# yeeus/GCI

Hardware: AMD Instinct MI355X
Metric: aligned Gbases/s through filter+depth pipeline (CHM13, 40x HiFi) (higher is better)
Workload: dtype int32

## Files before the change

### gci_amd/build.py

```python
from __future__ import annotations

import os
import subprocess

_HERE = os.path.dirname(os.path.abspath(__file__))
CSRC = os.path.join(_HERE, "csrc")
LIB = os.path.join(CSRC, "libgci_hip.so")
SOURCES = [os.path.join(CSRC, f) for f in ("api_ctx.hip", "k_filter.hip", "k_join.hip", "k_depth.hip", "k_track.hip", "k_bedgraph.hip", "k_hist.hip", "k_depth_parse.hip", "k_sdepth.hip", "k_deflate.hip", "k_depth_gz.hip", "k_paf.hip", "k_inflate.hip", "k_inflate_wave.hip", "k_records.hip", "k_pages.hip", "k_cover.hip", "k_shard.hip", "k_hbm.hip", "host_io.cpp", "staging.cpp")]
DEPS = SOURCES + [os.path.join(CSRC, "gci_common.h"), os.path.join(CSRC, "gci_ctx.hpp"), os.path.join(CSRC, "gci_wave.hpp"),
                  os.path.join(CSRC, "gci_text_tiles.hpp"), os.path.join(CSRC, "gci_crc_gf2.hpp"), os.path.join(CSRC, "gci_deflate_codes.hpp"),
                  os.path.join(_HERE, "..", "include", "gci_hip.h")]


def hipcc() -> str:
    for c in (os.environ.get("HIPCC"), "/opt/rocm/bin/hipcc", "hipcc"):
        if c and (os.path.sep not in c or os.path.exists(c)):
            return c
    raise RuntimeError("hipcc not found")


def needs_build() -> bool:
    if not os.path.exists(LIB):
        return True
    t = os.path.getmtime(LIB)
    return any(os.path.getmtime(d) > t for d in DEPS)
# ... 32 lines not shown
```

### gci_amd/csrc/api_ctx.hip

```cpp
#include "gci_ctx.hpp"
#include <stdlib.h>
#include <vector>

int gci_fail(gci_ctx* c, hipError_t e, const char* what)
{
    if (c) c->err = std::string(what) + ": " + hipGetErrorString(e);
    return GCI_E_HIP;
}

int gci_ensure(gci_ctx* ctx, DevBuf& b, size_t bytes)
{
    if (bytes <= b.cap) return GCI_OK;
    if (b.p) { HIPCHK(hipStreamSynchronize(ctx->stream)); HIPCHK(gci_dfree(b.p)); b.p = nullptr; b.cap = 0; }
    size_t want = bytes + bytes / 4 + 256;
    HIPCHK(gci_dmalloc(ctx->device, &b.p, want));
    b.cap = want;
    return GCI_OK;
}

int gci_upload_small(gci_ctx* ctx, void* d_dst, const void* h_src, size_t bytes)
{
    HIPCHK(hipStreamSynchronize(ctx->stream));
    if (bytes > ctx->h_pinned_cap) {
        if (ctx->h_pinned) HIPCHK(hipHostFree(ctx->h_pinned));
// ... 6 lines not shown
    memcpy(ctx->h_pinned, h_src, bytes);
    HIPCHK(hipMemcpyAsync(d_dst, ctx->h_pinned, bytes, hipMemcpyHostToDevice, ctx->stream));
    return GCI_OK;
}

extern "C" int gci_abi_version(void) { return GCI_ABI_VERSION; }

extern "C" int gci_ctx_create(int device, void* stream, int own_stream, gci_ctx** out)
{
    if (!out) return GCI_E_INVALID;
    gci_ctx* ctx = new (std::nothrow) gci_ctx();
    if (!ctx) return GCI_E_NOMEM;
    ctx->device = device;
    { const char* fd = getenv("GCI_FORCE_DENSE"); if (fd && fd[0] == '1') ctx->sparse_max = -1; }
    { const char* m = getenv("GCI_JOIN"); ctx->join_mode = m && m[0] == 'c' ? 1 : m && m[0] == 'p' ? 2 : 0; }
    { const char* g = getenv("GCI_PAGES_GRID"); const long n = g ? atol(g) : 0; ctx->pg_grid_cap = n > 0 && n < (1 << 20) ? (uint32_t)n : 0u; }
    hipError_t e = hipSetDevice(device);
    if (e != hipSuccess) { delete ctx; return GCI_E_HIP; }
    if (!own_stream) { ctx->stream = (hipStream_t)stream; }
    else {
        e = hipStreamCreateWithFlags(&ctx->stream, hipStreamNonBlocking);
        if (e != hipSuccess) { delete ctx; return GCI_E_HIP; }
        ctx->own_stream = true;
    }
    {
        uint32_t lut[TEXT_LUT];
        gci_text_lut_host(lut);
        if (gci_dmalloc(device, &ctx->text_lut.p, sizeof lut) != hipSuccess ||
            hipMemcpy(ctx->text_lut.p, lut, sizeof lut, hipMemcpyHostToDevice) != hipSuccess) {
            gci_ctx_destroy(ctx);
// ... 187 lines not shown
```

### gci_amd/csrc/gci_ctx.hpp

```cpp
#pragma once
#include <hip/hip_runtime.h>
#include <stdint.h>
#include <stdlib.h>
#include <string.h>
#include <string>
#include <vector>

#include "../../include/gci_hip.h"
#include "gci_common.h"
#include "gci_wave.hpp"

#define TILE GCI_TILE
#define TEXT_LUT 1000
#define BLOCK 256
static_assert(TILE == BLOCK * 16, "a tile is 16 elements per thread");

constexpr int GCI_RUN_MAX = 64;
constexpr uint32_t GCI_RUNS_WALK = 0xFFFFFFFFu;

struct DevBuf {
    void* p = nullptr;
    size_t cap = 0;
};

// ... 4 lines not shown
    std::string err;
    int32_t n_contigs = 0;
    std::vector<int64_t> len, off;
    std::vector<int64_t> tile_first;
    int64_t total = 0, n_tiles = 0;
    DevBuf d_len, d_off, d_tile_first;
    DevBuf tile_cd;
    DevBuf tile_carry;
    DevBuf evt_off;
    DevBuf d_tile_valid;
    DevBuf dense_flag;
    DevBuf dense_list;
    int32_t sparse_max = 62;
    bool join_dirty = false;
    int join_mode = 0;
    uint32_t k1_parity = 0;
    int cd_state = 0;
    int counted_flank = 0;
    bool count_deferred = false;
    DevBuf evp_items, evp_hist, evp_blk;
    DevBuf events;
    DevBuf blk_a, blk_b;
    DevBuf tile_sum;
    DevBuf tile_u32, tile_u64, blk_u64;
    uint32_t build_max_n = 0;
    int build_flank = 0;
    bool build_pending = false, build_text = false;
    bool build_runs_wanted = false;
    DevBuf build_nruns, build_runs;
    const void* build_runs_track = nullptr;
// ... 413 lines not shown
```

### gci_amd/csrc/k_join.hip

```cpp
#include "gci_ctx.hpp"
#include <stdlib.h>

struct JoinFiles {
    gci_join_file f[GCI_MAX_JOIN_FILES];
    int n;
};

#define SLOT_EMPTY 0xFFFFFFFFFFFFFFFFull

__device__ __forceinline__ const uint8_t* name_ptr(const gci_join_file& f, uint32_t idx)
{
    return f.d_name_base + f.d_name_off[idx] + f.name_delta;
}

__device__ __forceinline__ bool same_name(const JoinFiles& F, int fa, uint32_t ia, const gci_rec& a,
                                          unsigned long long owner)
{
    const int fb = (int)(owner >> 32);
    const uint32_t ib = (uint32_t)owner;
    const gci_rec& b = F.f[fb].d_recs[ib];
    if (a.name_hash != b.name_hash || a.name_len != b.name_len) return false;
    const uint8_t* pa = name_ptr(F.f[fa], ia);
    const uint8_t* pb = name_ptr(F.f[fb], ib);
    for (uint32_t i = 0; i < a.name_len; i++) if (pa[i] != pb[i]) return false;
// ... 145 lines not shown
        }
    }
}



struct __attribute__((aligned(16))) PartEntry {
    unsigned long long key;
    uint32_t idx;
    uint32_t meta;
    int32_t start, end, qlen;
    uint32_t name_off16;
};
static_assert(sizeof(PartEntry) == 32, "partition entry is 32 bytes");
#define PART_CHUNK 8192
#define PART_CONTIG_BITS 26
#define PART_KEY_MASK 0xFFFFFFFFFFFFull
#define PART_CMP_MASK 0x0FFFFFFFFFFFFFFFull
#define PART_MAX_NAME 4095u
#define PART_WIN (1ull << 63)
#define PART_NONE 0xFFFFFFFFu
struct PartFiles { uint32_t chunk_first[GCI_MAX_JOIN_FILES + 1]; };

__device__ __forceinline__ bool part_takes(const gci_rec& r)
{
    return (r.flags & GCI_REC_PASS) && !((uint32_t)r.contig >> PART_CONTIG_BITS) && r.name_len <= PART_MAX_NAME;
}

__device__ __forceinline__ void part_refuse(unsigned long long* status)
{
// ... 30 lines not shown
    return e;
}

__global__ __launch_bounds__(BLOCK) void k_part1_hist(JoinFiles F, PartFiles P, int shift, uint32_t n_bins, uint32_t n_chunks,
                                                      uint32_t* __restrict__ hist, uint32_t* __restrict__ reset_n_out,
                                                      unsigned long long* __restrict__ status)
{
    __shared__ uint32_t h[256];
    const uint32_t t = threadIdx.x, chunk = blockIdx.x;
    if (chunk == 0 && t == 0) *reset_n_out = 0;
    h[t] = 0;
    __syncthreads();
    const int f = part_file_of(P, F.n, chunk);
    const uint32_t i0 = (chunk - P.chunk_first[f]) * PART_CHUNK, n = F.f[f].n_recs;
    const gci_rec* __restrict__ recs = F.f[f].d_recs;
#pragma unroll 4
    for (int k = 0; k < PART_CHUNK / BLOCK; k++) {
        const uint32_t i = i0 + k * BLOCK + t;
        if (i < n) {
            const gci_rec r = recs[i];
            if (part_takes(r)) atomicAdd(&h[(uint32_t)((r.name_hash & PART_KEY_MASK) >> shift) & (n_bins - 1)], 1u);
            else if (r.flags & GCI_REC_PASS) part_refuse(status);
        }
    }
    __syncthreads();
    if (t < n_bins) hist[(size_t)t * n_chunks + chunk] = h[t];
}

#define SC_TILE 1024
#define SC_PER (SC_TILE / BLOCK)
struct ScatterLds {
    int4 stage[SC_TILE * 2];
    uint32_t tcnt[256], toff[256], gofs[256], cnt[256], base[256];
    uint32_t wtot[BLOCK / 64], total;
    uint8_t sbin[SC_TILE];
// ... 42 lines not shown
__global__ __launch_bounds__(BLOCK) void k_part1_scatter(JoinFiles F, PartFiles P, int shift, uint32_t n_bins, uint32_t n_chunks,
                                                         const uint32_t* __restrict__ off, PartEntry* __restrict__ out,
                                                         unsigned long long* __restrict__ status)
{
    __shared__ ScatterLds L;
    const uint32_t t = threadIdx.x, chunk = blockIdx.x;
    L.cnt[t] = 0; L.tcnt[t] = 0;
    L.base[t] = t < n_bins ? off[(size_t)t * n_chunks + chunk] : 0u;
    __syncthreads();
    const int f = part_file_of(P, F.n, chunk);
    const uint32_t i0 = (chunk - P.chunk_first[f]) * PART_CHUNK, n = F.f[f].n_recs;
    const gci_rec* __restrict__ recs = F.f[f].d_recs;
    const uint64_t* __restrict__ noff = F.f[f].d_name_off;
    const uint64_t delta = F.f[f].name_delta;
    for (uint32_t tile = 0; tile < PART_CHUNK && i0 + tile < n; tile += SC_TILE) {
        PartEntry e[SC_PER];
        int d[SC_PER];
#pragma unroll
        for (int k = 0; k < SC_PER; k++) {
            const uint32_t i = i0 + tile + k * BLOCK + t;
            d[k] = -1;
            e[k].key = 0; e[k].idx = 0; e[k].meta = 0; e[k].start = e[k].end = e[k].qlen = 0; e[k].name_off16 = 0;
            if (i < n) {
                const gci_rec r = recs[i];
                if (part_takes(r)) {
                    const uint64_t at = noff[i] + delta;
                    if (at >> 36) part_refuse(status);
                    e[k].key = (r.name_hash & PART_KEY_MASK) | ((unsigned long long)r.name_len << 48) | ((unsigned long long)(at & 15ull) << 60);
                    e[k].idx = i;
                    e[k].meta = (uint32_t)r.contig | ((uint32_t)f << PART_CONTIG_BITS) | ((r.flags & GCI_REC_HQ) ? 1u << 30 : 0u) |
                                ((r.flags & GCI_REC_NAME16) ? 1u << 31 : 0u);
                    e[k].start = r.start; e[k].end = r.end; e[k].qlen = r.qlen;
                    e[k].name_off16 = (uint32_t)(at >> 4);
                    d[k] = (int)((uint32_t)((e[k].key & PART_KEY_MASK) >> shift) & (n_bins - 1));
                }
            }
        }
        scatter_tile(L, e, d, n_bins, out, (int)t);
    }
}

__global__ __launch_bounds__(BLOCK) void k_part_mid(const uint32_t* __restrict__ off1, uint32_t n_bins, uint32_t n_chunks,
                                                    uint32_t* __restrict__ seg)
{
    __shared__ uint32_t s[257], c[257];
    const uint32_t t = threadIdx.x;
    if (t <= n_bins) s[t] = off1[(size_t)t * n_chunks];
    if (t == 0 && n_bins == 256) s[256] = off1[(size_t)256 * n_chunks];
    __syncthreads();
    if (t == 0) {
        uint32_t acc = 0;
        for (uint32_t d = 0; d < n_bins; d++) { c[d] = acc; acc += (s[d + 1] - s[d] + PART_CHUNK - 1) / PART_CHUNK; }
        c[n_bins] = acc;
    }
    __syncthreads();
    if (t <= n_bins) { seg[t] = s[t]; seg[n_bins + 1 + t] = c[t]; }
    if (t == 0 && n_bins == 256) { seg[256] = s[256]; seg[513] = c[256]; }
}

__device__ __forceinline__ bool part2_chunk(const uint32_t* sS, const uint32_t* sC, uint32_t n_seg, uint32_t w, uint32_t& j,
                                            uint32_t& k, uint32_t& a, uint32_t& b, uint32_t& nch)
{
    if (w >= sC[n_seg]) return false;
    uint32_t lo = 0, hi = n_seg;
    while (hi - lo > 1) { const uint32_t mid = (lo + hi) >> 1; if (sC[mid] <= w) lo = mid; else hi = mid; }
    j = lo; k = w - sC[j]; nch = sC[j + 1] - sC[j];
    a = sS[j] + k * PART_CHUNK;
    b = min(sS[j + 1], a + PART_CHUNK);
    return true;
}

__global__ __launch_bounds__(BLOCK) void k_part2_hist(const PartEntry* __restrict__ in, const uint32_t* __restrict__ seg,
                                                      uint32_t n_seg, int shift, uint32_t n_bins, uint32_t* __restrict__ hist)
{
    __shared__ uint32_t sS[257], sC[257], h[256];
    const uint32_t t = threadIdx.x, w = blockIdx.x;
    for (uint32_t i = t; i <= n_seg; i += BLOCK) { sS[i] = seg[i]; sC[i] = seg[n_seg + 1 + i]; }
    h[t] = 0;
    __syncthreads();
    uint32_t j, k, a, b, nch;
    if (!part2_chunk(sS, sC, n_seg, w, j, k, a, b, nch)) {
        if (t < n_bins) hist[(size_t)w * n_bins + t] = 0;
        return;
    }
    for (uint32_t i = a + t; i < b; i += BLOCK)
        atomicAdd(&h[(uint32_t)((in[i].key & PART_KEY_MASK) >> shift) & (n_bins - 1)], 1u);
    __syncthreads();
    if (t < n_bins) hist[(size_t)sC[j] * n_bins + (size_t)t * nch + k] = h[t];
}

__global__ __launch_bounds__(BLOCK) void k_part2_scatter(const PartEntry* __restrict__ in, const uint32_t* __restrict__ seg,
                                                         uint32_t n_seg, int shift, uint32_t n_bins,
                                                         const uint32_t* __restrict__ off, PartEntry* __restrict__ out)
{
    __shared__ ScatterLds L;
    __shared__ uint32_t sS[257], sC[257];
    const uint32_t t = threadIdx.x, w = blockIdx.x;
    for (uint32_t i = t; i <= n_seg; i += BLOCK) { sS[i] = seg[i]; sC[i] = seg[n_seg + 1 + i]; }
    L.cnt[t] = 0; L.tcnt[t] = 0;
    __syncthreads();
    uint32_t j, k, a, b, nch;
    if (!part2_chunk(sS, sC, n_seg, w, j, k, a, b, nch)) return;
    L.base[t] = t < n_bins ? off[(size_t)sC[j] * n_bins + (size_t)t * nch + k] : 0u;
    __syncthreads();
    for (uint32_t tile = a; tile < b; tile += SC_TILE) {
        PartEntry e[SC_PER];
        int d[SC_PER];
#pragma unroll
        for (int q = 0; q < SC_PER; q++) {
            const uint32_t i = tile + q * BLOCK + t;
            d[q] = -1;
            e[q].key = 0; e[q].idx = 0; e[q].meta = 0; e[q].start = e[q].end = e[q].qlen = 0; e[q].name_off16 = 0;
            if (i < b) {
                e[q] = load_entry(in + i);
                d[q] = (int)((uint32_t)((e[q].key & PART_KEY_MASK) >> shift) & (n_bins - 1));
            }
        }
        scatter_tile(L, e, d, n_bins, out, (int)t);
    }
}

__device__ __forceinline__ bool names_equal(const uint8_t* __restrict__ pa, const uint8_t* __restrict__ pb, uint32_t len)
{
    const uint32_t sa = (uint32_t)((uintptr_t)pa & 3u), sb = (uint32_t)((uintptr_t)pb & 3u);
    const uint32_t* __restrict__ qa = reinterpret_cast<const uint32_t*>(pa - sa);
    const uint32_t* __restrict__ qb = reinterpret_cast<const uint32_t*>(pb - sb);
    const uint32_t na = (sa + len + 3u) >> 2, nb = (sb + len + 3u) >> 2;
    uint32_t diff = 0;
    for (uint32_t w0 = 0; 4u * w0 < len; w0 += 8) {
        uint32_t a[9], b[9];
#pragma unroll
        for (int k = 0; k < 9; k++) {
// ... 19 lines not shown
    const uint32_t s = (uint32_t)((uintptr_t)pa & 15u);
    const uint4* __restrict__ qa = reinterpret_cast<const uint4*>(pa - s);
    const uint4* __restrict__ qb = reinterpret_cast<const uint4*>(pb - s);
    const uint32_t end = s + len;
    const uint4 z = make_uint4(0, 0, 0, 0);
    const uint4 a0 = qa[0], b0 = qb[0];
    const uint4 a1 = end > 16 ? qa[1] : z, b1 = end > 16 ? qb[1] : z;
    const uint4 a2 = end > 32 ? qa[2] : z, b2 = end > 32 ? qb[2] : z;
    uint32_t d = (s ? 0u : a0.x ^ b0.x) | (a0.y ^ b0.y) | (a0.z ^ b0.z) | (a0.w ^ b0.w);
    d |= (a1.x ^ b1.x) | (a1.y ^ b1.y) | (a1.z ^ b1.z) | (a1.w ^ b1.w);
    d |= (a2.x ^ b2.x) | (a2.y ^ b2.y) | (a2.z ^ b2.z) | (a2.w ^ b2.w);
    return d == 0;
}

struct PartJoinArgs {
    const PartEntry* in; const uint32_t* seg; const uint32_t* off2;
    uint32_t n_seg, n_bins2, slots, slot_shift;
};

template <bool CLAIM>
__device__ __forceinline__ uint32_t part_probe(unsigned long long* meta, uint32_t S, uint32_t slot_shift, const PartEntry& e, uint32_t i,
                                               const PartEntry* __restrict__ in, const JoinFiles& F, bool exact, uint16_t* used,
                                               uint32_t* s_used)
{
    const unsigned long long tag = e.key & 0xFFFFFFFFFFull;
    uint32_t slot = (uint32_t)((e.key & PART_KEY_MASK) >> slot_shift) & (S - 1);
    for (uint32_t probes = 0; probes < S; probes++) {
        unsigned long long m = meta[slot];
        if (m == SLOT_EMPTY) {
            if (!CLAIM) return PART_NONE;
            m = atomicCAS(meta + slot, SLOT_EMPTY, (tag << 24) | ((unsigned long long)i << 1));
            if (m == SLOT_EMPTY) {
                used[atomicAdd(s_used, 1u)] = (uint16_t)slot;
                return slot;
            }
        }
        if ((m >> 24) == tag) {
            if (!exact) return slot;
            const uint32_t c = (uint32_t)(m >> 1) & 0x7FFFFFu;
            if (c == i) return slot;
            const PartEntry ce = load_entry(in + c);
            if (((ce.key ^ e.key) & PART_CMP_MASK) == 0 &&
                names_equal(entry_name(F, e), entry_name(F, ce), (uint32_t)(e.key >> 48) & 0xFFFu))
                return slot;
        }
        slot = (slot + 1) & (S - 1);
    }
    return PART_NONE;
}

// ... 109 lines not shown
                else { s = ms; e = me; }
            } else have = false;
        } else {
            have = true; contig = r_contig; s = r.y; e = r.z;
        }
    }
    if (!have) return false;
    if (contig_map) { contig = contig_map[contig]; if (contig < 0) return false; }
    o.contig = contig; o.start = s; o.end = e; o.pad = 0;
    return true;
}

#ifndef PART_E
#define PART_E 2
#endif
#ifndef JB
#define JB 512
#endif
template <int FN>
__global__ __launch_bounds__(JB) __attribute__((amdgpu_waves_per_eu(4, 4))) void k_join_part(JoinFiles F, PartJoinArgs A, double ovlp_percent,
                                                     const int32_t* __restrict__ contig_map, gci_ivl* __restrict__ sparse,
                                                     uint32_t* __restrict__ bucket_cnt, uint32_t* __restrict__ bucket_lo,
                                                     unsigned long long* __restrict__ status, const CountArgs cnt)
{
    extern __shared__ __attribute__((aligned(16))) unsigned long long sm[];
    __shared__ uint32_t wtot[JB / 64];
    __shared__ uint32_t s_used, s_bad;
    __shared__ int64_t s_len[COUNT_LDS], s_tf[COUNT_LDS];
    const uint32_t S = A.slots;
    const int Fn = FN ? FN : F.n;
    unsigned long long* meta = sm;
    unsigned long long* cname = sm + S;
    unsigned long long* last = sm + 2 * (size_t)S;
    int4* pay = reinterpret_cast<int4*>(sm + 2 * (size_t)S + (size_t)S * Fn);
    uint16_t* used = reinterpret_cast<uint16_t*>(sm + 2 * (size_t)S + 3 * (size_t)S * Fn);
    const int t = threadIdx.x, lane = t & 63, wave = t >> 6;
    const uint32_t j = blockIdx.x / A.n_bins2, d = blockIdx.x % A.n_bins2;
    const uint32_t cj = A.seg[A.n_seg + 1 + j], nch = A.seg[A.n_seg + 2 + j] - cj;
    if (nch == 0) { if (t == 0) bucket_cnt[blockIdx.x] = 0u; return; }
    const uint32_t lo = A.off2[(size_t)cj * A.n_bins2 + (size_t)d * nch], hi = A.off2[(size_t)cj * A.n_bins2 + (size_t)(d + 1) * nch];
    if (t == 0) { bucket_cnt[blockIdx.x] = 0u; bucket_lo[blockIdx.x] = lo; }
    if (lo == hi) return;
    const bool tables_in_lds = cnt.tile_cd && cnt.n_contigs <= COUNT_LDS;
    if (tables_in_lds) for (int c = t; c < cnt.n_contigs; c += JB) { s_len[c] = cnt.len[c]; s_tf[c] = cnt.tile_first[c]; }
    const PartEntry* __restrict__ in = A.in + lo;
    const uint32_t n = hi - lo;
    if (n >> 23) {
        if (t == 0) part_refuse(status);
        return;
    }
    const uint32_t cmask = (1u << PART_CONTIG_BITS) - 1u;
    const bool in_regs = n <= PART_E * JB;
    PartEntry ent[PART_E];
    uint32_t slot_of[PART_E];
#pragma unroll
    for (int k = 0; k < PART_E; k++) {
        slot_of[k] = PART_NONE;
        const uint32_t i = (uint32_t)t + (uint32_t)k * JB;
        if (in_regs && i < n) ent[k] = load_entry(in + i);
        else { ent[k].key = 0; ent[k].idx = 0; ent[k].meta = 0; ent[k].start = ent[k].end = ent[k].qlen = 0; ent[k].name_off16 = 0; }
    }
    auto name_word = [](const PartEntry& e) -> unsigned long long {
        return (unsigned long long)e.name_off16 | ((e.key >> 60) << 32) | (((e.key >> 48) & 0xFFFull) << 36) |
               ((unsigned long long)((e.meta >> PART_CONTIG_BITS) & 15u) << 48) | ((unsigned long long)(e.meta >> 31) << 52);
    };
    auto insert = [&](const PartEntry& e, uint32_t i, bool exact) -> uint32_t {
        const uint32_t slot = part_probe<true>(meta, S, A.slot_shift, e, i, in, F, exact, used, &s_used);
        if (slot == PART_NONE) { part_refuse(status); return slot; }
        if (((uint32_t)(meta[slot] >> 1) & 0x7FFFFFu) == i) cname[slot] = name_word(e);
        const int file = (int)((e.meta >> PART_CONTIG_BITS) & 15u);
        const unsigned long long ord = (((unsigned long long)(e.meta & cmask) << 32) | e.idx) + 1ull;
        atomicMax(last + (size_t)slot * Fn + file, ord);
        if (Fn > 1 && (e.meta >> 30 & 1u)) atomicOr(meta + slot, 1ull);
        return slot;
    };
    auto settle = [&](const PartEntry& e, uint32_t i, uint32_t slot, bool exact) {
        const int file = (int)((e.meta >> PART_CONTIG_BITS) & 15u);
        const unsigned long long ord = (((unsigned long long)(e.meta & cmask) << 32) | e.idx) + 1ull;
        if (last[(size_t)slot * Fn + file] == ord) {
            last[(size_t)slot * Fn + file] = PART_WIN | i;
            pay[(size_t)slot * Fn + file] = make_int4((int)(e.meta & cmask), e.start, e.end, e.qlen);
        }
// ... 2 lines not shown
            const uint32_t len = (uint32_t)(e.key >> 48) & 0xFFFu;
            const uint8_t* cn = F.f[(cw >> 48) & 15u].d_name_base + (((cw & 0xFFFFFFFFull) << 4) | ((cw >> 32) & 15ull));
            const uint8_t* mn = entry_name(F, e);
            bool same;
            if (((uint32_t)(cw >> 36) & 0xFFFu) != len) same = false;
            else if ((e.meta >> 31) && ((cw >> 52) & 1ull) && len <= 44u && (((uintptr_t)mn ^ (uintptr_t)cn) & 15u) == 0)
                same = names_equal16(mn, cn, len);
            else same = names_equal(mn, cn, len);
            if (!same) s_bad = 1u;
        }
    };
    bool exact = false;
    for (;;) {
        for (uint32_t s = t; s < S; s += JB) meta[s] = SLOT_EMPTY;
        for (uint32_t s = t; s < S * (uint32_t)Fn; s += JB) last[s] = 0ull;
        if (t == 0) { s_used = 0; s_bad = 0; }
        __syncthreads();
        if (in_regs) {
#pragma unroll
            for (int k = 0; k < PART_E; k++) {
                const uint32_t i = (uint32_t)t + (uint32_t)k * JB;
                if (i < n) slot_of[k] = insert(ent[k], i, exact);
            }
        } else {
            for (uint32_t i = t; i < n; i += JB) insert(load_entry(in + i), i, exact);
        }
        __syncthreads();
        if (in_regs) {
#pragma unroll
            for (int k = 0; k < PART_E; k++) {
                const uint32_t i = (uint32_t)t + (uint32_t)k * JB;
                if (i < n && slot_of[k] != PART_NONE) settle(ent[k], i, slot_of[k], exact);
            }
        } else {
            for (uint32_t i = t; i < n; i += JB) {
                const PartEntry e = load_entry(in + i);
                const uint32_t slot = part_probe<false>(meta, S, A.slot_shift, e, i, in, F, exact, used, &s_used);
                if (slot != PART_NONE) settle(e, i, slot, exact);
            }
        }
        __syncthreads();
        if (exact || !s_bad) break;
        exact = true;
        __syncthreads();
    }
    auto fold_one = [&](const PartEntry& e, uint32_t i, uint32_t slot, gci_ivl& keep) -> bool {
        const int file = (int)((e.meta >> PART_CONTIG_BITS) & 15u);
        if (last[(size_t)slot * Fn + file] != (PART_WIN | i)) return false;
        for (int f = 0; f < file; f++) if (last[(size_t)slot * Fn + f] != 0) return false;
        return fold_from_entry<FN>(F, in, e, file, slot, last, pay, (meta[slot] & 1ull) != 0, ovlp_percent, contig_map, status, keep);
    };
    auto emit = [&](const gci_ivl& keep, uint32_t w) {
// ... 20 lines not shown
        uint32_t pre = inc - mine, all = 0;
#pragma unroll
        for (int w = 0; w < JB / 64; w++) { if (w < wave) pre += wtot[w]; all += wtot[w]; }
        if (t == 0) bucket_cnt[blockIdx.x] = all;
        uint32_t w = pre;
#pragma unroll
        for (int k = 0; k < PART_E; k++) if (ok[k]) emit(keep[k], w++);
    } else {
        uint32_t run = 0;
        for (uint32_t i0 = 0; i0 < n; i0 += JB) {
            const uint32_t i = i0 + t;
            gci_ivl keep;
            bool ok = false;
            if (i < n) {
                const PartEntry e = load_entry(in + i);
                const uint32_t slot = part_probe<false>(meta, S, A.slot_shift, e, i, in, F, exact, used, &s_used);
                ok = slot != PART_NONE && fold_one(e, i, slot, keep);
            }
            const unsigned long long bal = __ballot(ok);
            if (lane == 0) wtot[wave] = (uint32_t)__builtin_popcountll(bal);
            __syncthreads();
            uint32_t pre = (uint32_t)__builtin_popcountll(bal & ((1ull << lane) - 1ull)), all = 0;
#pragma unroll
            for (int w = 0; w < JB / 64; w++) { if (w < wave) pre += wtot[w]; all += wtot[w]; }
            if (ok) emit(keep, run + pre);
            run += all;
            __syncthreads();
        }
        if (t == 0) bucket_cnt[blockIdx.x] = run;
    }
}

__global__ __launch_bounds__(BLOCK) void k_join_gather(const gci_ivl* __restrict__ sparse, const uint32_t* __restrict__ bucket_cnt,
                                                       const uint32_t* __restrict__ bucket_lo, const uint32_t* __restrict__ off,
                                                       uint32_t n_buckets, gci_ivl* __restrict__ out, uint32_t cap, uint32_t* __restrict__ n_out)
{
    const uint32_t b = blockIdx.x * (BLOCK / 64) + (threadIdx.x >> 6), lane = threadIdx.x & 63;
    if (blockIdx.x == 0 && threadIdx.x == 0) *n_out = off[n_buckets];
    if (b >= n_buckets) return;
    const uint32_t c = bucket_cnt[b];
    if (!c) return;
    const gci_ivl* __restrict__ src = sparse + bucket_lo[b];
    const uint32_t o = off[b];
    for (uint32_t r = lane; r < c; r += 64) if (o + r < cap) out[o + r] = src[r];
}

static int name_join_partitioned(gci_ctx* ctx, const JoinFiles& F, uint64_t total, double ovlp_percent,
                                 const int32_t* d_contig_map, gci_ivl* d_out, uint32_t cap, uint32_t* d_n_out,
                                 uint64_t* d_status, const CountArgs& cnt, bool* done)
{
    *done = false;
    uint32_t S = 1024;
    while (S > 128 && (size_t)S * (16 + 24 * (size_t)F.n) > 65536) S >>= 1;
    uint64_t nb = 256;
    while (nb * S * 5 < total * 8) nb <<= 1;
    if (nb > 65536) return GCI_OK;
    int bits = 0;
    while ((1ull << bits) < nb) bits++;
    const int b1 = (bits + 1) / 2, b2 = bits - b1;
    const uint32_t B1 = 1u << b1, B2 = 1u << b2;
    int s_bits = 0;
    while ((1u << s_bits) < S) s_bits++;
    const int shift1 = 48 - b1, shift2 = 48 - b1 - b2, slot_shift = shift2 - s_bits;
    PartFiles P;
    uint32_t C1 = 0;
    for (int f = 0; f < F.n; f++) { P.chunk_first[f] = C1; C1 += (F.f[f].n_recs + PART_CHUNK - 1) / PART_CHUNK; }
    for (int f = F.n; f <= GCI_MAX_JOIN_FILES; f++) P.chunk_first[f] = C1;
    const uint32_t C2 = (uint32_t)(total / PART_CHUNK) + B1 + 1;
    const size_t n1 = (size_t)B1 * C1, n2 = (size_t)C2 * B2;
    GCI_TRY(gci_ensure(ctx, ctx->part_a, total * sizeof(PartEntry) + 16));
    GCI_TRY(gci_ensure(ctx, ctx->part_b, total * sizeof(PartEntry) + 16));
    GCI_TRY(gci_ensure(ctx, ctx->part_hist, (n1 + 1 + n2 + 1 + 2 * (size_t)B1 + 2) * 4 + 64));
    GCI_TRY(gci_ensure(ctx, ctx->part_blk, ((n1 > n2 ? n1 : n2) / TILE + 2) * 4));
    uint32_t* hist1 = (uint32_t*)ctx->part_hist.p;
    uint32_t* hist2 = hist1 + n1 + 1;
    uint32_t* seg = hist2 + n2 + 1;
    PartEntry* pa = (PartEntry*)ctx->part_a.p;
    PartEntry* pb = (PartEntry*)ctx->part_b.p;
    HIPCHK(hipMemsetAsync(d_status, 0xFF, 8, ctx->stream));
    {
        ProfScope _ps(ctx, GCI_PROF_PARTITION);
        hipLaunchKernelGGL(k_part1_hist, dim3(C1), dim3(BLOCK), 0, ctx->stream, F, P, shift1, B1, C1, hist1, d_n_out,
                           (unsigned long long*)d_status);
        LAUNCHCHK("k_part1_hist");
        int r = device_exclusive_scan<uint32_t, uint32_t>(ctx, hist1, hist1, (uint32_t*)ctx->part_blk.p, (int64_t)n1, true);
        if (r) return r;
        hipLaunchKernelGGL(k_part1_scatter, dim3(C1), dim3(BLOCK), 0, ctx->stream, F, P, shift1, B1, C1, (const uint32_t*)hist1, pa,
                           (unsigned long long*)d_status);
        LAUNCHCHK("k_part1_scatter");
        hipLaunchKernelGGL(k_part_mid, dim3(1), dim3(BLOCK), 0, ctx->stream, (const uint32_t*)hist1, B1, C1, seg);
        LAUNCHCHK("k_part_mid");
        hipLaunchKernelGGL(k_part2_hist, dim3(C2), dim3(BLOCK), 0, ctx->stream, (const PartEntry*)pa, (const uint32_t*)seg, B1,
                           shift2, B2, hist2);
        LAUNCHCHK("k_part2_hist");
        r = device_exclusive_scan<uint32_t, uint32_t>(ctx, hist2, hist2, (uint32_t*)ctx->part_blk.p, (int64_t)n2, true);
        if (r) return r;
        hipLaunchKernelGGL(k_part2_scatter, dim3(C2), dim3(BLOCK), 0, ctx->stream, (const PartEntry*)pa, (const uint32_t*)seg, B1,
                           shift2, B2, (const uint32_t*)hist2, pb);
        LAUNCHCHK("k_part2_scatter");
    }
    {
        ProfScope _ps(ctx, GCI_PROF_JOIN_PART);
        PartJoinArgs A;
        A.in = pb; A.seg = seg; A.off2 = hist2; A.n_seg = B1; A.n_bins2 = B2; A.slots = S; A.slot_shift = (uint32_t)slot_shift;
        const size_t lds = (size_t)S * (16 + 24 * (size_t)F.n) + (size_t)S * 2;
        const dim3 grid(B1 * B2), block(JB);
        const uint32_t NB = B1 * B2;
        GCI_TRY(gci_ensure(ctx, ctx->join_bucket, ((size_t)3 * NB + 2) * 4 + 64));
        uint32_t* bcnt = (uint32_t*)ctx->join_bucket.p;
        uint32_t* blo = bcnt + NB;
        uint32_t* boff = blo + NB;
        gci_ivl* sparse = (gci_ivl*)pa;
        static_assert(sizeof(gci_ivl) <= sizeof(PartEntry), "the sparse intervals fit the partition buffer");
        const void* kfn = F.n == 1 ? (const void*)k_join_part<1> : F.n == 2 ? (const void*)k_join_part<2> : F.n == 3 ? (const void*)k_join_part<3>
                        : F.n == 4 ? (const void*)k_join_part<4> : (const void*)k_join_part<0>;
        HIPCHK(hipFuncSetAttribute(kfn, hipFuncAttributeMaxDynamicSharedMemorySize, (int)lds));
        switch (F.n) {
        case 1: hipLaunchKernelGGL((k_join_part<1>), grid, block, lds, ctx->stream, F, A, ovlp_percent, d_contig_map, sparse, bcnt, blo, (unsigned long long*)d_status, cnt); break;
        case 2: hipLaunchKernelGGL((k_join_part<2>), grid, block, lds, ctx->stream, F, A, ovlp_percent, d_contig_map, sparse, bcnt, blo, (unsigned long long*)d_status, cnt); break;
        case 3: hipLaunchKernelGGL((k_join_part<3>), grid, block, lds, ctx->stream, F, A, ovlp_percent, d_contig_map, sparse, bcnt, blo, (unsigned long long*)d_status, cnt); break;
        case 4: hipLaunchKernelGGL((k_join_part<4>), grid, block, lds, ctx->stream, F, A, ovlp_percent, d_contig_map, sparse, bcnt, blo, (unsigned long long*)d_status, cnt); break;
        default: hipLaunchKernelGGL((k_join_part<0>), grid, block, lds, ctx->stream, F, A, ovlp_percent, d_contig_map, sparse, bcnt, blo, (unsigned long long*)d_status, cnt); break;
        }
        LAUNCHCHK("k_join_part");
        int r2 = device_exclusive_scan<uint32_t, uint32_t>(ctx, bcnt, boff, (uint32_t*)ctx->part_blk.p, (int64_t)NB, true);
        if (r2) return r2;
        hipLaunchKernelGGL(k_join_gather, dim3((NB + BLOCK / 64 - 1) / (BLOCK / 64)), dim3(BLOCK), 0, ctx->stream, (const gci_ivl*)sparse,
                           (const uint32_t*)bcnt, (const uint32_t*)blo, (const uint32_t*)boff, NB, d_out, cap, d_n_out);
        LAUNCHCHK("k_join_gather");
    }
    *done = true;
    return GCI_OK;
}

static int name_join_impl(gci_ctx* ctx, const gci_join_file* h_files, int n_files, double ovlp_percent,
                          const int32_t* d_contig_map, gci_ivl* d_out, uint32_t cap, uint32_t* d_n_out,
                          uint64_t* d_status, const CountArgs& cnt)
{
    if (!ctx || !h_files || n_files < 1 || n_files > GCI_MAX_JOIN_FILES || !d_n_out || !d_status || (cap && !d_out))
        return GCI_E_INVALID;
    JoinFiles F;
    memset(&F, 0, sizeof F);
    F.n = n_files;
// ... 241 lines not shown
```

Before: 25150.

## Plan smaller join hash tables, batch partition loads, precompute bucket ranges

Adds a join planner that picks a smaller 512-slot table with 256-thread blocks when the bucket count allows, which doubles the number of buckets. A new GCI_JOIN_TABLE=l option restores the old large-table plan. The partition histogram and scatter kernels now batch or prefetch their record loads into registers to raise memory-level parallelism. Bucket [lo,hi) ranges are written by k_part_mid and k_part2_scatter, so the join kernel no longer recomputes them from segment offsets. The used-slot list is dropped and the contig tables move into dynamic LDS, at the cost of more registers and more, smaller blocks.

After: 25420 (median of 6 runs). 1.01x the previous value.

```diff
diff --git a/gci_amd/build.py b/gci_amd/build.py
--- a/gci_amd/build.py
+++ b/gci_amd/build.py
@@ -8,7 +8,7 @@
 LIB = os.path.join(CSRC, "libgci_hip.so")
 SOURCES = [os.path.join(CSRC, f) for f in ("api_ctx.hip", "k_filter.hip", "k_join.hip", "k_depth.hip", "k_track.hip", "k_bedgraph.hip", "k_hist.hip", "k_depth_parse.hip", "k_sdepth.hip", "k_deflate.hip", "k_depth_gz.hip", "k_paf.hip", "k_inflate.hip", "k_inflate_wave.hip", "k_records.hip", "k_pages.hip", "k_cover.hip", "k_shard.hip", "k_hbm.hip", "host_io.cpp", "staging.cpp")]
 DEPS = SOURCES + [os.path.join(CSRC, "gci_common.h"), os.path.join(CSRC, "gci_ctx.hpp"), os.path.join(CSRC, "gci_wave.hpp"),
-                  os.path.join(CSRC, "gci_text_tiles.hpp"), os.path.join(CSRC, "gci_crc_gf2.hpp"), os.path.join(CSRC, "gci_deflate_codes.hpp"),
+                  os.path.join(CSRC, "gci_text_tiles.hpp"), os.path.join(CSRC, "gci_crc_gf2.hpp"), os.path.join(CSRC, "gci_deflate_codes.hpp"), os.path.join(CSRC, "gci_join_plan.hpp"),
                   os.path.join(_HERE, "..", "include", "gci_hip.h")]
 
 
diff --git a/gci_amd/csrc/api_ctx.hip b/gci_amd/csrc/api_ctx.hip
--- a/gci_amd/csrc/api_ctx.hip
+++ b/gci_amd/csrc/api_ctx.hip
@@ -44,6 +44,7 @@
     ctx->device = device;
     { const char* fd = getenv("GCI_FORCE_DENSE"); if (fd && fd[0] == '1') ctx->sparse_max = -1; }
     { const char* m = getenv("GCI_JOIN"); ctx->join_mode = m && m[0] == 'c' ? 1 : m && m[0] == 'p' ? 2 : 0; }
+    { const char* m = getenv("GCI_JOIN_TABLE"); ctx->join_table_large = m && m[0] == 'l'; }
     { const char* g = getenv("GCI_PAGES_GRID"); const long n = g ? atol(g) : 0; ctx->pg_grid_cap = n > 0 && n < (1 << 20) ? (uint32_t)n : 0u; }
     hipError_t e = hipSetDevice(device);
     if (e != hipSuccess) { delete ctx; return GCI_E_HIP; }
diff --git a/gci_amd/csrc/gci_ctx.hpp b/gci_amd/csrc/gci_ctx.hpp
--- a/gci_amd/csrc/gci_ctx.hpp
+++ b/gci_amd/csrc/gci_ctx.hpp
@@ -42,6 +42,7 @@
     int32_t sparse_max = 62;
     bool join_dirty = false;
     int join_mode = 0;
+    bool join_table_large = false;
     uint32_t k1_parity = 0;
     int cd_state = 0;
     int counted_flank = 0;
diff --git a/gci_amd/csrc/gci_join_plan.hpp b/gci_amd/csrc/gci_join_plan.hpp
--- /dev/null
+++ b/gci_amd/csrc/gci_join_plan.hpp
@@ -0,0 +1,37 @@
+#pragma once
+#include <cstddef>
+#include <cstdint>
+
+struct JoinPlan {
+    bool partition;
+    uint32_t slots;
+    uint32_t threads;
+    uint32_t b1, b2;
+    size_t lds;
+};
+
+inline uint64_t join_plan_buckets(uint64_t total, uint32_t S)
+{
+    uint64_t nb = 256;
+    while (nb * S * 5 < total * 8) nb <<= 1;
+    return nb;
+}
+
+inline JoinPlan join_plan(uint64_t total, int n_files, bool force_large)
+{
+    JoinPlan p;
+    uint32_t S_large = 1024;
+    while (S_large > 128 && (size_t)S_large * (16 + 24 * (size_t)n_files) > 65536) S_large >>= 1;
+    const uint32_t S_small = S_large < 512 ? S_large : 512;
+    const bool small = !force_large && join_plan_buckets(total, S_small) <= 65536;
+    p.slots = small ? S_small : S_large;
+    p.threads = small ? 256 : 512;
+    const uint64_t nb = join_plan_buckets(total, p.slots);
+    p.partition = nb <= 65536;
+    int bits = 0;
+    while ((1ull << bits) < nb) bits++;
+    p.b1 = (uint32_t)(bits + 1) / 2;
+    p.b2 = (uint32_t)bits - p.b1;
+    p.lds = (size_t)p.slots * (16 + 24 * (size_t)n_files);
+    return p;
+}
diff --git a/gci_amd/csrc/k_join.hip b/gci_amd/csrc/k_join.hip
--- a/gci_amd/csrc/k_join.hip
+++ b/gci_amd/csrc/k_join.hip
@@ -1,4 +1,5 @@
 #include "gci_ctx.hpp"
+#include "gci_join_plan.hpp"
 #include <stdlib.h>
 
 struct JoinFiles {
@@ -183,6 +184,8 @@
 };
 static_assert(sizeof(PartEntry) == 32, "partition entry is 32 bytes");
 #define PART_CHUNK 8192
+#define H1_BATCH 8
+static_assert(offsetof(gci_rec, mapq) == 28 && offsetof(gci_rec, flags) == 29 && offsetof(gci_rec, name_len) == 30, "k_part1_hist reads them as one word");
 #define PART_CONTIG_BITS 26
 #define PART_KEY_MASK 0xFFFFFFFFFFFFull
 #define PART_CMP_MASK 0x0FFFFFFFFFFFFFFFull
@@ -243,11 +246,23 @@
     const int f = part_file_of(P, F.n, chunk);
     const uint32_t i0 = (chunk - P.chunk_first[f]) * PART_CHUNK, n = F.f[f].n_recs;
     const gci_rec* __restrict__ recs = F.f[f].d_recs;
-#pragma unroll 4
-    for (int k = 0; k < PART_CHUNK / BLOCK; k++) {
-        const uint32_t i = i0 + k * BLOCK + t;
-        if (i < n) {
-            const gci_rec r = recs[i];
+    for (int k0 = 0; k0 < PART_CHUNK / BLOCK; k0 += H1_BATCH) {
+        unsigned long long hash[H1_BATCH];
+        int32_t contig[H1_BATCH];
+        uint32_t tail[H1_BATCH];
+#pragma unroll
+        for (int k = 0; k < H1_BATCH; k++) {
+            const uint32_t i = min(i0 + (k0 + k) * BLOCK + t, n - 1);
+            hash[k] = recs[i].name_hash;
+            contig[k] = recs[i].contig;
+            tail[k] = reinterpret_cast<const uint32_t*>(recs + i)[7];
+        }
+#pragma unroll
+        for (int k = 0; k < H1_BATCH; k++) {
+            if (i0 + (k0 + k) * BLOCK + t >= n) continue;
+            gci_rec r;
+            r.name_hash = hash[k]; r.contig = contig[k];
+            r.flags = (uint8_t)(tail[k] >> 8); r.name_len = (uint16_t)(tail[k] >> 16);
             if (part_takes(r)) atomicAdd(&h[(uint32_t)((r.name_hash & PART_KEY_MASK) >> shift) & (n_bins - 1)], 1u);
             else if (r.flags & GCI_REC_PASS) part_refuse(status);
         }
@@ -320,6 +335,14 @@
     const uint64_t* __restrict__ noff = F.f[f].d_name_off;
     const uint64_t delta = F.f[f].name_delta;
     for (uint32_t tile = 0; tile < PART_CHUNK && i0 + tile < n; tile += SC_TILE) {
+        gci_rec rr[SC_PER];
+        uint64_t ra[SC_PER];
+#pragma unroll
+        for (int k = 0; k < SC_PER; k++) {
+            const uint32_t i = min(i0 + tile + k * BLOCK + t, n - 1);
+            rr[k] = recs[i];
+            ra[k] = noff[i];
+        }
         PartEntry e[SC_PER];
         int d[SC_PER];
 #pragma unroll
@@ -328,9 +351,9 @@
             d[k] = -1;
             e[k].key = 0; e[k].idx = 0; e[k].meta = 0; e[k].start = e[k].end = e[k].qlen = 0; e[k].name_off16 = 0;
             if (i < n) {
-                const gci_rec r = recs[i];
+                const gci_rec r = rr[k];
                 if (part_takes(r)) {
-                    const uint64_t at = noff[i] + delta;
+                    const uint64_t at = ra[k] + delta;
                     if (at >> 36) part_refuse(status);
                     e[k].key = (r.name_hash & PART_KEY_MASK) | ((unsigned long long)r.name_len << 48) | ((unsigned long long)(at & 15ull) << 60);
                     e[k].idx = i;
@@ -347,7 +370,7 @@
 }
 
 __global__ __launch_bounds__(BLOCK) void k_part_mid(const uint32_t* __restrict__ off1, uint32_t n_bins, uint32_t n_chunks,
-                                                    uint32_t* __restrict__ seg)
+                                                    uint32_t* __restrict__ seg, uint32_t n_bins2, uint32_t* __restrict__ range)
 {
     __shared__ uint32_t s[257], c[257];
     const uint32_t t = threadIdx.x;
@@ -362,6 +385,9 @@
     __syncthreads();
     if (t <= n_bins) { seg[t] = s[t]; seg[n_bins + 1 + t] = c[t]; }
     if (t == 0 && n_bins == 256) { seg[256] = s[256]; seg[513] = c[256]; }
+    if (t < n_bins && s[t + 1] == s[t])
+        for (uint32_t d = 0; d < n_bins2; d++) range[(size_t)t * n_bins2 + d] = s[t];
+    if (t == 0) range[(size_t)n_bins * n_bins2] = s[n_bins];
 }
 
 __device__ __forceinline__ bool part2_chunk(const uint32_t* sS, const uint32_t* sC, uint32_t n_seg, uint32_t w, uint32_t& j,
@@ -389,15 +415,22 @@
         if (t < n_bins) hist[(size_t)w * n_bins + t] = 0;
         return;
     }
-    for (uint32_t i = a + t; i < b; i += BLOCK)
-        atomicAdd(&h[(uint32_t)((in[i].key & PART_KEY_MASK) >> shift) & (n_bins - 1)], 1u);
+    for (uint32_t base = a; base < b; base += H1_BATCH * BLOCK) {
+        unsigned long long key[H1_BATCH];
+#pragma unroll
+        for (int q = 0; q < H1_BATCH; q++) key[q] = in[min(base + q * BLOCK + t, b - 1)].key;
+#pragma unroll
+        for (int q = 0; q < H1_BATCH; q++)
+            if (base + q * BLOCK + t < b) atomicAdd(&h[(uint32_t)((key[q] & PART_KEY_MASK) >> shift) & (n_bins - 1)], 1u);
+    }
     __syncthreads();
     if (t < n_bins) hist[(size_t)sC[j] * n_bins + (size_t)t * nch + k] = h[t];
 }
 
 __global__ __launch_bounds__(BLOCK) void k_part2_scatter(const PartEntry* __restrict__ in, const uint32_t* __restrict__ seg,
                                                          uint32_t n_seg, int shift, uint32_t n_bins,
-                                                         const uint32_t* __restrict__ off, PartEntry* __restrict__ out)
+                                                         const uint32_t* __restrict__ off, PartEntry* __restrict__ out,
+                                                         uint32_t* __restrict__ range)
 {
     __shared__ ScatterLds L;
     __shared__ uint32_t sS[257], sC[257];
@@ -407,8 +440,16 @@
     __syncthreads();
     uint32_t j, k, a, b, nch;
     if (!part2_chunk(sS, sC, n_seg, w, j, k, a, b, nch)) return;
-    L.base[t] = t < n_bins ? off[(size_t)sC[j] * n_bins + (size_t)t * nch + k] : 0u;
-    __syncthreads();
+    const uint32_t first = t < n_bins ? off[(size_t)sC[j] * n_bins + (size_t)t * nch + k] : 0u;
+    L.base[t] = first;
+    if (k == 0 && t < n_bins) range[(size_t)j * n_bins + t] = first;
+    __syncthreads();
+    PartEntry ne[SC_PER];
+    auto fetch = [&](uint32_t tile) {
+#pragma unroll
+        for (int q = 0; q < SC_PER; q++) ne[q] = load_entry(in + min(tile + q * BLOCK + t, b - 1));
+    };
+    fetch(a);
     for (uint32_t tile = a; tile < b; tile += SC_TILE) {
         PartEntry e[SC_PER];
         int d[SC_PER];
@@ -418,10 +459,11 @@
             d[q] = -1;
             e[q].key = 0; e[q].idx = 0; e[q].meta = 0; e[q].start = e[q].end = e[q].qlen = 0; e[q].name_off16 = 0;
             if (i < b) {
-                e[q] = load_entry(in + i);
+                e[q] = ne[q];
                 d[q] = (int)((uint32_t)((e[q].key & PART_KEY_MASK) >> shift) & (n_bins - 1));
             }
         }
+        fetch(tile + SC_TILE);
         scatter_tile(L, e, d, n_bins, out, (int)t);
     }
 }
@@ -471,14 +513,13 @@
 }
 
 struct PartJoinArgs {
-    const PartEntry* in; const uint32_t* seg; const uint32_t* off2;
-    uint32_t n_seg, n_bins2, slots, slot_shift;
+    const PartEntry* in; const uint32_t* range;
+    uint32_t slots, slot_shift;
 };
 
 template <bool CLAIM>
 __device__ __forceinline__ uint32_t part_probe(unsigned long long* meta, uint32_t S, uint32_t slot_shift, const PartEntry& e, uint32_t i,
-                                               const PartEntry* __restrict__ in, const JoinFiles& F, bool exact, uint16_t* used,
-                                               uint32_t* s_used)
+                                               const PartEntry* __restrict__ in, const JoinFiles& F, bool exact)
 {
     const unsigned long long tag = e.key & 0xFFFFFFFFFFull;
     uint32_t slot = (uint32_t)((e.key & PART_KEY_MASK) >> slot_shift) & (S - 1);
@@ -487,10 +528,7 @@
         if (m == SLOT_EMPTY) {
             if (!CLAIM) return PART_NONE;
             m = atomicCAS(meta + slot, SLOT_EMPTY, (tag << 24) | ((unsigned long long)i << 1));
-            if (m == SLOT_EMPTY) {
-                used[atomicAdd(s_used, 1u)] = (uint16_t)slot;
-                return slot;
-            }
+            if (m == SLOT_EMPTY) return slot;
         }
         if ((m >> 24) == tag) {
             if (!exact) return slot;
@@ -630,39 +668,32 @@
 #ifndef PART_E
 #define PART_E 2
 #endif
-#ifndef JB
-#define JB 512
-#endif
-template <int FN>
+template <int FN, int JB>
 __global__ __launch_bounds__(JB) __attribute__((amdgpu_waves_per_eu(4, 4))) void k_join_part(JoinFiles F, PartJoinArgs A, double ovlp_percent,
                                                      const int32_t* __restrict__ contig_map, gci_ivl* __restrict__ sparse,
-                                                     uint32_t* __restrict__ bucket_cnt, uint32_t* __restrict__ bucket_lo,
+                                                     uint32_t* __restrict__ bucket_cnt,
                                                      unsigned long long* __restrict__ status, const CountArgs cnt)
 {
     extern __shared__ __attribute__((aligned(16))) unsigned long long sm[];
     __shared__ uint32_t wtot[JB / 64];
-    __shared__ uint32_t s_used, s_bad;
-    __shared__ int64_t s_len[COUNT_LDS], s_tf[COUNT_LDS];
+    __shared__ uint32_t s_bad;
     const uint32_t S = A.slots;
     const int Fn = FN ? FN : F.n;
     unsigned long long* meta = sm;
     unsigned long long* cname = sm + S;
     unsigned long long* last = sm + 2 * (size_t)S;
     int4* pay = reinterpret_cast<int4*>(sm + 2 * (size_t)S + (size_t)S * Fn);
-    uint16_t* used = reinterpret_cast<uint16_t*>(sm + 2 * (size_t)S + 3 * (size_t)S * Fn);
+    int64_t* s_len = reinterpret_cast<int64_t*>(sm + 2 * (size_t)S + 3 * (size_t)S * Fn);
+    int64_t* s_tf = s_len + COUNT_LDS;
     const int t = threadIdx.x, lane = t & 63, wave = t >> 6;
-    const uint32_t j = blockIdx.x / A.n_bins2, d = blockIdx.x % A.n_bins2;
-    const uint32_t cj = A.seg[A.n_seg + 1 + j], nch = A.seg[A.n_seg + 2 + j] - cj;
-    if (nch == 0) { if (t == 0) bucket_cnt[blockIdx.x] = 0u; return; }
-    const uint32_t lo = A.off2[(size_t)cj * A.n_bins2 + (size_t)d * nch], hi = A.off2[(size_t)cj * A.n_bins2 + (size_t)(d + 1) * nch];
-    if (t == 0) { bucket_cnt[blockIdx.x] = 0u; bucket_lo[blockIdx.x] = lo; }
-    if (lo == hi) return;
+    const uint32_t lo = A.range[blockIdx.x], hi = A.range[blockIdx.x + 1];
+    if (lo == hi) { if (t == 0) bucket_cnt[blockIdx.x] = 0u; return; }
     const bool tables_in_lds = cnt.tile_cd && cnt.n_contigs <= COUNT_LDS;
     if (tables_in_lds) for (int c = t; c < cnt.n_contigs; c += JB) { s_len[c] = cnt.len[c]; s_tf[c] = cnt.tile_first[c]; }
     const PartEntry* __restrict__ in = A.in + lo;
     const uint32_t n = hi - lo;
     if (n >> 23) {
-        if (t == 0) part_refuse(status);
+        if (t == 0) { bucket_cnt[blockIdx.x] = 0u; part_refuse(status); }
         return;
     }
     const uint32_t cmask = (1u << PART_CONTIG_BITS) - 1u;
@@ -681,7 +712,7 @@
                ((unsigned long long)((e.meta >> PART_CONTIG_BITS) & 15u) << 48) | ((unsigned long long)(e.meta >> 31) << 52);
     };
     auto insert = [&](const PartEntry& e, uint32_t i, bool exact) -> uint32_t {
-        const uint32_t slot = part_probe<true>(meta, S, A.slot_shift, e, i, in, F, exact, used, &s_used);
+        const uint32_t slot = part_probe<true>(meta, S, A.slot_shift, e, i, in, F, exact);
         if (slot == PART_NONE) { part_refuse(status); return slot; }
         if (((uint32_t)(meta[slot] >> 1) & 0x7FFFFFu) == i) cname[slot] = name_word(e);
         const int file = (int)((e.meta >> PART_CONTIG_BITS) & 15u);
@@ -714,7 +745,7 @@
     for (;;) {
         for (uint32_t s = t; s < S; s += JB) meta[s] = SLOT_EMPTY;
         for (uint32_t s = t; s < S * (uint32_t)Fn; s += JB) last[s] = 0ull;
-        if (t == 0) { s_used = 0; s_bad = 0; }
+        if (t == 0) s_bad = 0;
         __syncthreads();
         if (in_regs) {
 #pragma unroll
@@ -735,7 +766,7 @@
         } else {
             for (uint32_t i = t; i < n; i += JB) {
                 const PartEntry e = load_entry(in + i);
-                const uint32_t slot = part_probe<false>(meta, S, A.slot_shift, e, i, in, F, exact, used, &s_used);
+                const uint32_t slot = part_probe<false>(meta, S, A.slot_shift, e, i, in, F, exact);
                 if (slot != PART_NONE) settle(e, i, slot, exact);
             }
         }
@@ -786,7 +817,7 @@
             bool ok = false;
             if (i < n) {
                 const PartEntry e = load_entry(in + i);
-                const uint32_t slot = part_probe<false>(meta, S, A.slot_shift, e, i, in, F, exact, used, &s_used);
+                const uint32_t slot = part_probe<false>(meta, S, A.slot_shift, e, i, in, F, exact);
                 ok = slot != PART_NONE && fold_one(e, i, slot, keep);
             }
             const unsigned long long bal = __ballot(ok);
@@ -804,7 +835,7 @@
 }
 
 __global__ __launch_bounds__(BLOCK) void k_join_gather(const gci_ivl* __restrict__ sparse, const uint32_t* __restrict__ bucket_cnt,
-                                                       const uint32_t* __restrict__ bucket_lo, const uint32_t* __restrict__ off,
+                                                       const uint32_t* __restrict__ range, const uint32_t* __restrict__ off,
                                                        uint32_t n_buckets, gci_ivl* __restrict__ out, uint32_t cap, uint32_t* __restrict__ n_out)
 {
     const uint32_t b = blockIdx.x * (BLOCK / 64) + (threadIdx.x >> 6), lane = threadIdx.x & 63;
@@ -812,9 +843,27 @@
     if (b >= n_buckets) return;
     const uint32_t c = bucket_cnt[b];
     if (!c) return;
-    const gci_ivl* __restrict__ src = sparse + bucket_lo[b];
+    const gci_ivl* __restrict__ src = sparse + range[b];
     const uint32_t o = off[b];
     for (uint32_t r = lane; r < c; r += 64) if (o + r < cap) out[o + r] = src[r];
+}
+
+template <int JB>
+static int launch_join_part(gci_ctx* ctx, uint32_t n_buckets, size_t lds, const JoinFiles& F, const PartJoinArgs& A, double ovlp_percent,
+                            const int32_t* d_contig_map, gci_ivl* sparse, uint32_t* bcnt, uint64_t* d_status, const CountArgs& cnt)
+{
+    const dim3 grid(n_buckets), block(JB);
+    const void* kfn = F.n == 1 ? (const void*)k_join_part<1, JB> : F.n == 2 ? (const void*)k_join_part<2, JB>
+                    : F.n == 3 ? (const void*)k_join_part<3, JB> : F.n == 4 ? (const void*)k_join_part<4, JB> : (const void*)k_join_part<0, JB>;
+    HIPCHK(hipFuncSetAttribute(kfn, hipFuncAttributeMaxDynamicSharedMemorySize, (int)lds));
+    switch (F.n) {
+    case 1: hipLaunchKernelGGL((k_join_part<1, JB>), grid, block, lds, ctx->stream, F, A, ovlp_percent, d_contig_map, sparse, bcnt, (unsigned long long*)d_status, cnt); break;
+    case 2: hipLaunchKernelGGL((k_join_part<2, JB>), grid, block, lds, ctx->stream, F, A, ovlp_percent, d_contig_map, sparse, bcnt, (unsigned long long*)d_status, cnt); break;
+    case 3: hipLaunchKernelGGL((k_join_part<3, JB>), grid, block, lds, ctx->stream, F, A, ovlp_percent, d_contig_map, sparse, bcnt, (unsigned long long*)d_status, cnt); break;
+    case 4: hipLaunchKernelGGL((k_join_part<4, JB>), grid, block, lds, ctx->stream, F, A, ovlp_percent, d_contig_map, sparse, bcnt, (unsigned long long*)d_status, cnt); break;
+    default: hipLaunchKernelGGL((k_join_part<0, JB>), grid, block, lds, ctx->stream, F, A, ovlp_percent, d_contig_map, sparse, bcnt, (unsigned long long*)d_status, cnt); break;
+    }
+    return GCI_OK;
 }
 
 static int name_join_partitioned(gci_ctx* ctx, const JoinFiles& F, uint64_t total, double ovlp_percent,
@@ -822,15 +871,11 @@
                                  uint64_t* d_status, const CountArgs& cnt, bool* done)
 {
     *done = false;
-    uint32_t S = 1024;
-    while (S > 128 && (size_t)S * (16 + 24 * (size_t)F.n) > 65536) S >>= 1;
-    uint64_t nb = 256;
-    while (nb * S * 5 < total * 8) nb <<= 1;
-    if (nb > 65536) return GCI_OK;
-    int bits = 0;
-    while ((1ull << bits) < nb) bits++;
-    const int b1 = (bits + 1) / 2, b2 = bits - b1;
-    const uint32_t B1 = 1u << b1, B2 = 1u << b2;
+    const JoinPlan plan = join_plan(total, F.n, ctx->join_table_large);
+    if (!plan.partition) return GCI_OK;
+    const uint32_t S = plan.slots;
+    const int b1 = (int)plan.b1, b2 = (int)plan.b2;
+    const uint32_t B1 = 1u << b1, B2 = 1u << b2, NB = B1 * B2;
     int s_bits = 0;
     while ((1u << s_bits) < S) s_bits++;
     const int shift1 = 48 - b1, shift2 = 48 - b1 - b2, slot_shift = shift2 - s_bits;
@@ -849,6 +894,10 @@
     uint32_t* seg = hist2 + n2 + 1;
     PartEntry* pa = (PartEntry*)ctx->part_a.p;
     PartEntry* pb = (PartEntry*)ctx->part_b.p;
+    GCI_TRY(gci_ensure(ctx, ctx->join_bucket, ((size_t)3 * NB + 2) * 4 + 64));
+    uint32_t* bcnt = (uint32_t*)ctx->join_bucket.p;
+    uint32_t* range = bcnt + NB;
+    uint32_t* boff = range + NB + 1;
     HIPCHK(hipMemsetAsync(d_status, 0xFF, 8, ctx->stream));
     {
         ProfScope _ps(ctx, GCI_PROF_PARTITION);
@@ -860,7 +909,7 @@
         hipLaunchKernelGGL(k_part1_scatter, dim3(C1), dim3(BLOCK), 0, ctx->stream, F, P, shift1, B1, C1, (const uint32_t*)hist1, pa,
                            (unsigned long long*)d_status);
         LAUNCHCHK("k_part1_scatter");
-        hipLaunchKernelGGL(k_part_mid, dim3(1), dim3(BLOCK), 0, ctx->stream, (const uint32_t*)hist1, B1, C1, seg);
+        hipLaunchKernelGGL(k_part_mid, dim3(1), dim3(BLOCK), 0, ctx->stream, (const uint32_t*)hist1, B1, C1, seg, B2, range);
         LAUNCHCHK("k_part_mid");
         hipLaunchKernelGGL(k_part2_hist, dim3(C2), dim3(BLOCK), 0, ctx->stream, (const PartEntry*)pa, (const uint32_t*)seg, B1,
                            shift2, B2, hist2);
@@ -868,37 +917,25 @@
         r = device_exclusive_scan<uint32_t, uint32_t>(ctx, hist2, hist2, (uint32_t*)ctx->part_blk.p, (int64_t)n2, true);
         if (r) return r;
         hipLaunchKernelGGL(k_part2_scatter, dim3(C2), dim3(BLOCK), 0, ctx->stream, (const PartEntry*)pa, (const uint32_t*)seg, B1,
-                           shift2, B2, (const uint32_t*)hist2, pb);
+                           shift2, B2, (const uint32_t*)hist2, pb, range);
         LAUNCHCHK("k_part2_scatter");
     }
     {
         ProfScope _ps(ctx, GCI_PROF_JOIN_PART);
         PartJoinArgs A;
-        A.in = pb; A.seg = seg; A.off2 = hist2; A.n_seg = B1; A.n_bins2 = B2; A.slots = S; A.slot_shift = (uint32_t)slot_shift;
-        const size_t lds = (size_t)S * (16 + 24 * (size_t)F.n) + (size_t)S * 2;
-        const dim3 grid(B1 * B2), block(JB);
-        const uint32_t NB = B1 * B2;
-        GCI_TRY(gci_ensure(ctx, ctx->join_bucket, ((size_t)3 * NB + 2) * 4 + 64));
-        uint32_t* bcnt = (uint32_t*)ctx->join_bucket.p;
-        uint32_t* blo = bcnt + NB;
-        uint32_t* boff = blo + NB;
+        A.in = pb; A.range = range; A.slots = S; A.slot_shift = (uint32_t)slot_shift;
+        const size_t lds = plan.lds + (cnt.tile_cd && cnt.n_contigs <= COUNT_LDS ? (size_t)2 * COUNT_LDS * sizeof(int64_t) : 0);
         gci_ivl* sparse = (gci_ivl*)pa;
         static_assert(sizeof(gci_ivl) <= sizeof(PartEntry), "the sparse intervals fit the partition buffer");
-        const void* kfn = F.n == 1 ? (const void*)k_join_part<1> : F.n == 2 ? (const void*)k_join_part<2> : F.n == 3 ? (const void*)k_join_part<3>
-                        : F.n == 4 ? (const void*)k_join_part<4> : (const void*)k_join_part<0>;
-        HIPCHK(hipFuncSetAttribute(kfn, hipFuncAttributeMaxDynamicSharedMemorySize, (int)lds));
-        switch (F.n) {
-        case 1: hipLaunchKernelGGL((k_join_part<1>), grid, block, lds, ctx->stream, F, A, ovlp_percent, d_contig_map, sparse, bcnt, blo, (unsigned long long*)d_status, cnt); break;
-        case 2: hipLaunchKernelGGL((k_join_part<2>), grid, block, lds, ctx->stream, F, A, ovlp_percent, d_contig_map, sparse, bcnt, blo, (unsigned long long*)d_status, cnt); break;
-        case 3: hipLaunchKernelGGL((k_join_part<3>), grid, block, lds, ctx->stream, F, A, ovlp_percent, d_contig_map, sparse, bcnt, blo, (unsigned long long*)d_status, cnt); break;
-        case 4: hipLaunchKernelGGL((k_join_part<4>), grid, block, lds, ctx->stream, F, A, ovlp_percent, d_contig_map, sparse, bcnt, blo, (unsigned long long*)d_status, cnt); break;
-        default: hipLaunchKernelGGL((k_join_part<0>), grid, block, lds, ctx->stream, F, A, ovlp_percent, d_contig_map, sparse, bcnt, blo, (unsigned long long*)d_status, cnt); break;
-        }
+        int r1;
+        if (plan.threads == 256) r1 = launch_join_part<256>(ctx, NB, lds, F, A, ovlp_percent, d_contig_map, sparse, bcnt, d_status, cnt);
+        else r1 = launch_join_part<512>(ctx, NB, lds, F, A, ovlp_percent, d_contig_map, sparse, bcnt, d_status, cnt);
+        if (r1) return r1;
         LAUNCHCHK("k_join_part");
         int r2 = device_exclusive_scan<uint32_t, uint32_t>(ctx, bcnt, boff, (uint32_t*)ctx->part_blk.p, (int64_t)NB, true);
         if (r2) return r2;
         hipLaunchKernelGGL(k_join_gather, dim3((NB + BLOCK / 64 - 1) / (BLOCK / 64)), dim3(BLOCK), 0, ctx->stream, (const gci_ivl*)sparse,
-                           (const uint32_t*)bcnt, (const uint32_t*)blo, (const uint32_t*)boff, NB, d_out, cap, d_n_out);
+                           (const uint32_t*)bcnt, (const uint32_t*)range, (const uint32_t*)boff, NB, d_out, cap, d_n_out);
         LAUNCHCHK("k_join_gather");
     }
     *done = true;
```
